# i4Ds/whisper-finetune

Hardware: AMD Instinct MI355X
Metric: audio-seconds/sec training throughput, whisper-large-v3 bf16 (higher is better)
Workload: dtype bf16; 1 GPU; whisper-large-v3 full fine-tune, AdamW, bf16 MFMA / fp32 master weights, 96 synthetic 30 s clips per GPU per step, decoder S=128, log-mel + SpecAugment on GPU, label smoothing 0.1, clip 1.0, local accumulation 1 (global window = 1); timed loop = model_utils.train_step; global_batch=96, seq_len=128, parallelism=dp1

## Files before the change

### include/wft.h

```cpp
#ifndef WFT_H
#define WFT_H

#include <stdint.h>

#ifdef __cplusplus
extern "C" {
#endif

typedef enum {
  WFT_OK = 0,
  WFT_ERR_ARG = -1,
  WFT_ERR_LAUNCH = -2,
  WFT_ERR_UNSUPPORTED = -3
} wft_status;

typedef uint16_t wft_bf16;

const char* wft_last_error(void);
const char* wft_version(void);

int wft_cast_f32_bf16(const float* src, wft_bf16* dst, int64_t n, void* stream);
int wft_cast_bf16_f32(const wft_bf16* src, float* dst, int64_t n, void* stream);
int wft_cast_pad_transpose_f32_bf16(const float* src, int64_t rows, int64_t cols,
                                    wft_bf16* dst, wft_bf16* dst_t,
// ... 90 lines not shown
int wft_gemm_nt_rank_pair_bf16(const wft_gemm_args* args0, const wft_gemm_args* args1, void* stream);
int wft_gemm_tn_rank_pair_bf16(const wft_gemm_args* args0, const wft_gemm_args* args1, void* stream);
int64_t wft_gemm_tn_workspace_bytes(const wft_gemm_args* args);

typedef struct {
  const wft_bf16* q; int64_t ldq; int64_t q_bs;
  const wft_bf16* k; int64_t ldk; int64_t k_bs;
  const wft_bf16* v; int64_t ldv; int64_t v_bs;
  wft_bf16* o; int64_t ldo; int64_t o_bs;
  float* lse;
  int B; int H; int Tq; int Tk; int causal; float scale;
  const wft_bf16* d_o; int64_t lddo; int64_t do_bs;
  float* delta;
  wft_bf16* dq; int64_t lddq; int64_t dq_bs;
  wft_bf16* dk; int64_t lddk; int64_t dk_bs;
  wft_bf16* dv; int64_t lddv; int64_t dv_bs;
  float* dq_colsum; float* dv_colsum; float* colsum_ws;
  int launch_mode; int variant; int q_prescaled;
} wft_attn_args;
int wft_attn_fwd_bf16(const wft_attn_args* args, void* stream);
int wft_attn_bwd_bf16(const wft_attn_args* args, void* stream);
int64_t wft_attn_bwd_colsum_workspace_bytes(const wft_attn_args* args);
int wft_attn_variant(const wft_attn_args* args, int which);

int wft_embed_fwd(const int64_t* tokens, const float* emb, const float* pos,
                  wft_bf16* out, int64_t B, int64_t S, int d, int64_t V, void* stream);
int wft_embed_bwd(const int64_t* tokens, const wft_bf16* dout, float* demb, float* dpos,
                  int64_t B, int64_t S, int d, int64_t V, void* stream);

int wft_ce_fwd(const wft_bf16* logits, int64_t ld, const int64_t* targets,
               int64_t rows, int64_t V, float label_smoothing,
               float* row_loss, float* row_lse, float* stats, int64_t* argmax,
               void* stream);
int wft_ce_bwd(const wft_bf16* logits, int64_t ld, const int64_t* targets,
               int64_t rows, int64_t V, float label_smoothing,
               const float* row_lse, const float* stats, const float* gscale,
               wft_bf16* dlogits, void* stream);

int wft_token_stats(const wft_bf16* logits, int64_t ld, const int64_t* targets,
                    int64_t rows, int64_t V, float* out4, int64_t* argmax, void* stream);

typedef struct {
  const wft_bf16* q; int64_t ldq;
  const wft_bf16* k_new; const wft_bf16* v_new; int64_t ld_new;
  wft_bf16* k_cache; wft_bf16* v_cache; int64_t ld_cache; int64_t cache_bs;
  wft_bf16* o; int64_t ldo;
// ... 146 lines not shown
```

### whisper-finetune_amd/csrc/attn.hip

```cpp
#include "attn_common.h"

static void attn_fill(const wft_attn_args* a, AttnP& p) {
  p.q = a->q; p.ldq = a->ldq; p.q_bs = a->q_bs;
  p.k = a->k; p.ldk = a->ldk; p.k_bs = a->k_bs;
  p.v = a->v; p.ldv = a->ldv; p.v_bs = a->v_bs;
  p.o = a->o; p.ldo = a->ldo; p.o_bs = a->o_bs;
  p.lse = a->lse;
  p.B = a->B; p.H = a->H; p.Tq = a->Tq; p.Tk = a->Tk; p.causal = a->causal;
  p.scale = a->scale;
  p.qpre = a->q_prescaled ? 1 : 0;
  p.c = p.qpre ? 1.0f : a->scale * LOG2E;
  p.ls = p.qpre ? LN2 : a->scale;
  p.d_o = a->d_o; p.lddo = a->lddo; p.do_bs = a->do_bs;
  p.delta = a->delta;
  p.dq = a->dq; p.lddq = a->lddq; p.dq_bs = a->dq_bs;
  p.dk = a->dk; p.lddk = a->lddk; p.dk_bs = a->dk_bs;
  p.dv = a->dv; p.lddv = a->lddv; p.dv_bs = a->dv_bs;
  p.cs_q = nullptr; p.cs_v = nullptr;
  static const int xcd_on = [] { const char* e = wft_dev_getenv("WFT_ATTN_XCD"); return e ? atoi(e) : 1; }();
  p.xcd = xcd_on;
}

#define ATT_CS_CHUNKS 32
__global__ __launch_bounds__(256) void attn_colsum_reduce_kernel(const float* partial0, long nrows0, float* out0,
// ... 17 lines not shown

#define ATT_ALIGNED(ptr, ld, bs) ((((uintptr_t)(ptr)) & 15) == 0 && ((ld) % 8) == 0 && ((bs) % 8) == 0)
static int attn_check(const wft_attn_args* a, bool bwd, const char* who, const char* align_msg) {
  WFT_CHECK_ARG_AS(who, a && a->q && a->k && a->v && a->o && a->lse &&
                            (!bwd || (a->d_o && a->delta && a->dq && a->dk && a->dv)),
                   "null pointer");
  WFT_CHECK_ARG_AS(who, a->B >= 1 && a->H >= 1 && a->Tq >= 1 && a->Tk >= 1, "bad shape");
  WFT_CHECK_ARG_AS(who, ATT_ALIGNED(a->q, a->ldq, a->q_bs) && ATT_ALIGNED(a->k, a->ldk, a->k_bs) &&
                            ATT_ALIGNED(a->v, a->ldv, a->v_bs) && ATT_ALIGNED(a->o, a->ldo, a->o_bs) &&
                            (!bwd || (ATT_ALIGNED(a->d_o, a->lddo, a->do_bs) && ATT_ALIGNED(a->dq, a->lddq, a->dq_bs) &&
                                      ATT_ALIGNED(a->dk, a->lddk, a->dk_bs) && ATT_ALIGNED(a->dv, a->lddv, a->dv_bs))),
                   align_msg);
  WFT_CHECK_ARG_AS(who, !a->causal || a->Tq == a->Tk, "causal attention needs Tq == Tk");
  if (!bwd) return WFT_OK;
  WFT_CHECK_ARG_AS(who, a->scale > 0.f, "scale must be positive (the row constants are -lse / scale)");
  WFT_CHECK_ARG_AS(who, (!a->dq_colsum && !a->dv_colsum && !a->colsum_ws) || (a->dq_colsum && a->dv_colsum && a->colsum_ws),
                   "dq_colsum, dv_colsum and colsum_ws go together");
  return WFT_OK;
}

static int g_attn_persistent = [] { const char* e = getenv("WFT_ATTN_PERSISTENT"); return (e && e[0] == '0') ? 0 : 1; }();
struct AttnPlan {
  bool fwd_pipe = false;
  bool dq4w = false, dkdv4w = false;
  unsigned fwd_grid = 0, dq_grid = 0, dkdv_grid = 0;
  long rows_q = 0, rows_v = 0, cs_q = 0, cs_v = 0, mid_q = 0, mid_v = 0;
  int64_t colsum_bytes = 0;
};
static unsigned attn_persistent_grid(const wft_attn_args* a, int rows, int wgs_env) {
  const bool persistent = g_attn_persistent != 0 && a->launch_mode != 1;
  const long items = (long)((rows + 255) / 256) * a->H * a->B;
  long wgs = wgs_env > 0 ? wgs_env : (persistent ? wft_num_cus() : items);
  if (wgs > items) wgs = items;
  if (((long)a->H * a->B) % 8 == 0 && wgs >= 8) wgs -= wgs % 8;
  return (unsigned)wgs;
}
static AttnPlan attn_plan(const wft_attn_args* a) {
  AttnPlan pl;
  if (!a) return pl;
  static const int dkdv_wgs_env = [] { const char* e = wft_dev_getenv("WFT_DKDV_WGS"); return e ? atoi(e) : 0; }();
  pl.fwd_pipe = wft_fwd_pipe_eligible(a);
  pl.dq4w = wft_dq4w_eligible(a);
  pl.dkdv4w = wft_dkdv4w_eligible(a);
  const unsigned grid_q = (unsigned)(((a->Tq + 127) / 128) * a->H * a->B), grid_k = (unsigned)(((a->Tk + 127) / 128) * a->H * a->B);
  pl.fwd_grid = grid_q;
  pl.dq_grid = pl.dq4w ? attn_persistent_grid(a, a->Tq, 0) : grid_q;
  pl.dkdv_grid = pl.dkdv4w ? attn_persistent_grid(a, a->Tk, dkdv_wgs_env) : grid_k;
  const long n = (long)a->H * 64;
  pl.rows_q = (long)a->B * ((a->Tq + 31) / 32);
  pl.rows_v = (long)a->B * ((a->Tk + 31) / 32);
  pl.cs_v = pl.rows_q * n;
  pl.mid_q = pl.cs_v + pl.rows_v * n;
  pl.mid_v = pl.mid_q + (long)ATT_CS_CHUNKS * n;
  pl.colsum_bytes = (pl.mid_v + (int64_t)ATT_CS_CHUNKS * n) * (int64_t)sizeof(float);
  return pl;
}

extern "C" int64_t wft_attn_bwd_colsum_workspace_bytes(const wft_attn_args* a) { return attn_plan(a).colsum_bytes; }

extern "C" int wft_attn_variant(const wft_attn_args* a, int which) {
  if (!a) return WFT_ERR_ARG;
  const AttnPlan pl = attn_plan(a);
  if (which == 0) return pl.fwd_pipe ? 2 : 1;
  if (which == 1) return pl.dq4w ? 4 : 8;
  if (which == 2) return pl.dkdv4w ? 4 : 8;
  return WFT_ERR_ARG;
}

extern "C" int wft_attn_fwd_bf16(const wft_attn_args* a, void* stream) {
  if (const int rc = attn_check(a, false, __func__, "q/k/v/o need 16-byte aligned bases and strides that are multiples of 8")) return rc;
  AttnP p;
  attn_fill(a, p);
  const AttnPlan pl = attn_plan(a);
  wft_attn_fwd_launch(p, pl.fwd_pipe, dim3(pl.fwd_grid), (hipStream_t)stream);
  WFT_CHECK_LAUNCH();
  return WFT_OK;
}

extern "C" int wft_attn_bwd_bf16(const wft_attn_args* a, void* stream) {
  if (const int rc = attn_check(a, true, __func__, "tensors need 16-byte aligned bases and strides that are multiples of 8")) return rc;
  AttnP p;
  attn_fill(a, p);
  const AttnPlan pl = attn_plan(a);
  if (a->colsum_ws) {
    p.cs_q = a->colsum_ws + pl.cs_q;
    p.cs_v = a->colsum_ws + pl.cs_v;
  }
  hipStream_t s = (hipStream_t)stream;
  int rc = WFT_OK;
  if (pl.dq4w) rc = wft_dq4w_launch(p, dim3(pl.dq_grid), s);
  else wft_attn_dq8w_launch(p, dim3(pl.dq_grid), s);
  if (rc != WFT_OK) return rc;
  rc = pl.dkdv4w ? wft_dkdv4w_launch(p, dim3(pl.dkdv_grid), s) : wft_attn_dkdv8w_launch(p, dim3(pl.dkdv_grid), s);
  if (rc != WFT_OK) return rc;
  if (p.cs_q) {
    const int n = a->H * 64;
    float* mid_q = a->colsum_ws + pl.mid_q;
// ... 10 lines not shown
```

### whisper-finetune_amd/csrc/attn_common.h

```cpp
#pragma once
#include "common.h"
#include "gemm_common.h"
#include <stdlib.h>
#include <string.h>
#define ATT_NEG (-1.0e30f)
#define ATT_TAU 8.0f
#define LOG2E 1.4426950408889634f
#define LN2 0.6931471805599453f

struct AttnP {
  const unsigned short* q; long ldq, q_bs;
  const unsigned short* k; long ldk, k_bs;
  const unsigned short* v; long ldv, v_bs;
  unsigned short* o; long ldo, o_bs;
  float* lse;
  int B, H, Tq, Tk, causal;
  float scale;
  const unsigned short* d_o; long lddo, do_bs;
  float* delta;
  unsigned short* dq; long lddq, dq_bs;
  unsigned short* dk; long lddk, dk_bs;
  unsigned short* dv; long lddv, dv_bs;
  float* cs_q;
  float* cs_v;
// ... 205 lines not shown
template <int N>
__device__ __forceinline__ float w4_acc() {
  float x;
  asm volatile("v_accvgpr_read_b32 %0, a[%1]" : "=v"(x) : "i"(N));
  return x;
}
template <int BASE>
__device__ __forceinline__ f32x16 w4_get16() {
  f32x16 v;
  v[0] = w4_acc<BASE>(); v[1] = w4_acc<BASE + 1>(); v[2] = w4_acc<BASE + 2>(); v[3] = w4_acc<BASE + 3>();
  v[4] = w4_acc<BASE + 4>(); v[5] = w4_acc<BASE + 5>(); v[6] = w4_acc<BASE + 6>(); v[7] = w4_acc<BASE + 7>();
  v[8] = w4_acc<BASE + 8>(); v[9] = w4_acc<BASE + 9>(); v[10] = w4_acc<BASE + 10>(); v[11] = w4_acc<BASE + 11>();
  v[12] = w4_acc<BASE + 12>(); v[13] = w4_acc<BASE + 13>(); v[14] = w4_acc<BASE + 14>(); v[15] = w4_acc<BASE + 15>();
  return v;
}

static inline bool attn_offsets_fit32(const wft_attn_args* a) {
  const long lim = 0x7fffffffL;
  return (long)(a->Tq + 256) * a->ldq * 2 < lim && (long)(a->Tq + 256) * a->lddo * 2 < lim && (long)(a->Tk + 256) * a->ldk * 2 < lim &&
         (long)(a->Tk + 256) * a->ldv * 2 < lim;
}
bool wft_fwd_pipe_eligible(const wft_attn_args* a);
void wft_attn_fwd_launch(const AttnP& p, bool pipe, dim3 grid, hipStream_t s);
void wft_attn_dq8w_launch(const AttnP& p, dim3 grid, hipStream_t s);
int wft_attn_dkdv8w_launch(const AttnP& p, dim3 grid, hipStream_t s);
bool wft_dq4w_eligible(const wft_attn_args* a);
int wft_dq4w_launch(const AttnP& p, dim3 grid, hipStream_t s);
bool wft_dkdv4w_eligible(const wft_attn_args* a);
int wft_dkdv4w_launch(const AttnP& p, dim3 grid, hipStream_t s);
```

### whisper-finetune_amd/whisper_finetune/engine/kernels.py

```python
from __future__ import annotations

import ctypes as C
import math
from typing import Optional

import torch

from . import lib as L

BF16 = torch.bfloat16
F32 = torch.float32

PROFILE_NT = None


def _p(t: Optional[torch.Tensor]):
    return C.c_void_p(0 if t is None else t.data_ptr())


def _chk(t: torch.Tensor, dtype, name: str):
    if t.dtype != dtype:
        raise TypeError(f"{name}: expected {dtype}, got {t.dtype}")
    if not t.is_cuda:
        raise L.WftError(f"{name}: libwft kernels need CUDA/HIP tensors (got {t.device}); there is no CPU path")
# ... 191 lines not shown
    need_ws = want_params or want_colsum
    ws = torch.empty(lib.wft_layernorm_bwd_workspace(rows, cols), dtype=torch.uint8, device=x.device) if need_ws else None
    dx = torch.empty_like(x)
    dgamma = torch.empty(cols, dtype=F32, device=x.device) if want_params else None
    dbeta = torch.empty(cols, dtype=F32, device=x.device) if want_params else None
    dxs = torch.empty(cols, dtype=F32, device=x.device) if want_colsum else None
    if mask is not None and len(mask) == 2:
        rpb, span = mask
        _chk_flag(span, 4, "span")
        L.check(lib.wft_layernorm_bwd_dspan(_p(dy), _p(x), _p(gamma), _p(mean), _p(rstd), _p(dres), _p(dx), _p(dgamma), _p(dbeta),
                                            _p(dxs), _p(ws), rows, cols, int(rpb), _p(span), L.stream_ptr()), "wft_layernorm_bwd_dspan")
    else:
        rpb, t0, t1, c0, c1 = mask if mask is not None else (0, 0, 0, 0, 0)
        L.check(
                lib.wft_layernorm_bwd(_p(dy), _p(x), _p(gamma), _p(mean), _p(rstd), _p(dres), _p(dx), _p(dgamma), _p(dbeta),
                                      _p(dxs), _p(ws), rows, cols, rpb, t0, t1, c0, c1, L.stream_ptr()),
            "wft_layernorm_bwd",
        )
    if want_colsum:
        return dx, dgamma, dbeta, dxs
    return dx, dgamma, dbeta


VARIANT = {"nt": 0, "tn": 0, "fwd": 0, "dq": 0, "dkdv": 0}
LAUNCH_OVERRIDE = [None]
LAUNCH_PERSISTENT, LAUNCH_PER_TILE = 0, 1


def set_variant(which: str, v: int) -> int:
    old = VARIANT[which]
    if v >= 0:
        VARIANT[which] = 1 if v else 0
    return old


def _launch(launch: int) -> int:
    o = LAUNCH_OVERRIDE[0]
    return int(launch) if o is None else int(o)


def _attn_variant_bits() -> int:
    return VARIANT["fwd"] | (VARIANT["dq"] << 1) | (VARIANT["dkdv"] << 2)


def gemm_nt(a, b, *, M=None, N=None, K=None, lda=None, ldb=None, out=None, out_f32=False, accumulate=False,
            bias=None, residual=None, aux=None, epilogue=L.EPI_NONE, alpha=1.0, batch=1,
            strideA=0, strideB=0, strideC=0, strideR=0, strideAux=0, ldc=None,
            valid_rows_period=0, valid_rows=0, residual_first=False, ldaux=None, ldr=None, beta=1.0, colsum=None, p_valid=0,
            launch=0, _args_only=False):
    _chk(a, BF16, "A"); _chk(b, BF16, "B")
    if M is None:
        M = a.shape[0]
    if K is None:
        K = a.shape[-1]
    if N is None:
        N = b.shape[0]
    if lda is None:
        lda = a.stride(-2) if a.dim() >= 2 else K
    if ldb is None:
        ldb = b.stride(-2)
    if out is None:
        out = torch.empty((batch * M, N) if batch > 1 else (M, N), dtype=F32 if out_f32 else BF16, device=a.device)
        if batch > 1 and strideC == 0:
            strideC = M * N
    if ldc is None:
# ... 212 lines not shown

def _tn_workspace(device, nbytes: int, slot: str = "tn") -> torch.Tensor:
    key = (device.type, device.index, slot)
    ws = _TN_WS.get(key)
    if ws is None or ws.numel() < nbytes:
        ws = torch.empty(max(nbytes, 64 << 20), dtype=torch.uint8, device=device)
        _TN_WS[key] = ws
    return ws


def _grant_workspace(args, query: str, device, slot: str) -> int:
    need = getattr(L.load(), query)(C.byref(args))
    if need > 0:
        ws = _tn_workspace(device, need, slot=slot)
        args.workspace, args.workspace_bytes = ws.data_ptr(), ws.numel()
    return need


def _attn_view(t: torch.Tensor):
    assert t.dim() == 3 and t.stride(2) == 1
    return t.data_ptr(), t.stride(1), t.stride(0)


def attn_fwd(q, k, v, n_head: int, causal: bool, scale: float, q_prescaled: bool = False, o=None, lse=None):
    for n, t in (("q", q), ("k", k), ("v", v)):
        _chk(t, BF16, n)
    B, Tq, D = q.shape
    Tk = k.shape[1]
    assert D == n_head * 64, "head_dim must be 64"
    if o is None:
        o = torch.empty((B, Tq, D), dtype=BF16, device=q.device)
    else:
        _chk(o, BF16, "o")
        assert o.shape == (B, Tq, D)
    if lse is None:
        lse = torch.empty((B, n_head, Tq), dtype=F32, device=q.device)
    else:
        _chk(lse, F32, "lse")
        assert lse.shape == (B, n_head, Tq) and lse.is_contiguous()
    a = L.AttnArgs()
    a.q, a.ldq, a.q_bs = _attn_view(q)
    a.k, a.ldk, a.k_bs = _attn_view(k)
    a.v, a.ldv, a.v_bs = _attn_view(v)
    a.o, a.ldo, a.o_bs = _attn_view(o)
    a.lse = lse.data_ptr()
    a.B, a.H, a.Tq, a.Tk, a.causal, a.scale = B, n_head, Tq, Tk, int(causal), scale
    a.variant, a.q_prescaled = _attn_variant_bits(), int(bool(q_prescaled))
    L.check(L.load().wft_attn_fwd_bf16(C.byref(a), L.stream_ptr()), "wft_attn_fwd_bf16")
    return o, lse


def attn_bwd(q, k, v, o, lse, do, n_head: int, causal: bool, scale: float, dq=None, dk=None, dv=None, colsums=None,
             q_prescaled: bool = False, launch: int = 0):
    B, Tq, D = q.shape
    Tk = k.shape[1]
    _chk(do, BF16, "do")
    if do.stride(2) != 1:
        do = do.contiguous()
    dq = torch.empty((B, Tq, D), dtype=BF16, device=q.device) if dq is None else dq
    dk = torch.empty((B, Tk, D), dtype=BF16, device=q.device) if dk is None else dk
    dv = torch.empty((B, Tk, D), dtype=BF16, device=q.device) if dv is None else dv
    delta = torch.empty((2, B, n_head, Tq), dtype=F32, device=q.device)
    a = L.AttnArgs()
    a.q, a.ldq, a.q_bs = _attn_view(q)
    a.k, a.ldk, a.k_bs = _attn_view(k)
    a.v, a.ldv, a.v_bs = _attn_view(v)
    a.o, a.ldo, a.o_bs = _attn_view(o)
    a.lse = lse.data_ptr()
    a.B, a.H, a.Tq, a.Tk, a.causal, a.scale = B, n_head, Tq, Tk, int(causal), scale
    a.d_o, a.lddo, a.do_bs = _attn_view(do)
# ... 693 lines not shown
```

### whisper-finetune_amd/whisper_finetune/engine/lib.py

```python
from __future__ import annotations

import ctypes as C
import os
from pathlib import Path

_PKG_ROOT = Path(__file__).resolve().parents[2]
LIB_PATH = Path(os.environ.get("WFT_LIB", _PKG_ROOT / "libwft.so"))

c_i64 = C.c_int64
c_vp = C.c_void_p


class GemmArgs(C.Structure):

    _fields_ = [
        ("A", c_vp), ("lda", c_i64), ("strideA", c_i64),
        ("B", c_vp), ("ldb", c_i64), ("strideB", c_i64),
        ("C", c_vp), ("ldc", c_i64), ("strideC", c_i64), ("c_is_f32", C.c_int), ("accumulate", C.c_int),
        ("bias", c_vp),
        ("residual", c_vp), ("ldr", c_i64), ("strideR", c_i64),
        ("aux", c_vp), ("ldaux", c_i64), ("strideAux", c_i64),
        ("epilogue", C.c_int), ("alpha", C.c_float),
        ("M", c_i64), ("N", c_i64), ("K", c_i64), ("batch", C.c_int),
        ("valid_rows_period", C.c_int), ("valid_rows", C.c_int),
# ... 139 lines not shown
    "wft_layernorm_bwd_dspan": [c_vp, c_vp, c_vp, c_vp, c_vp, c_vp, c_vp, c_vp, c_vp, c_vp, c_vp, c_i64, C.c_int,
                                C.c_int, c_vp, c_vp],
    "wft_gemm_nt_bf16": [C.POINTER(GemmArgs), c_vp],
    "wft_gemm_nt_variant": [C.POINTER(GemmArgs)],
    "wft_gemm_tn_segments_ok": [C.POINTER(GemmArgs)],
    "wft_gemm_nt_colsum_workspace_bytes": [C.POINTER(GemmArgs)],
    "wft_gemm_nt_splitk_workspace_bytes": [C.POINTER(GemmArgs)],
    "wft_gemm_nt_aux8_bytes": [C.POINTER(GemmArgs)],
    "wft_gemm_nt_stream_bf16": [C.POINTER(GemmArgs), c_vp],
    "wft_gemm_nt_stream_ok": [C.POINTER(GemmArgs)],
    "wft_gemm_nt_stream_workspace_bytes": [C.POINTER(GemmArgs)],
    "wft_gemm_nt_stream_q8": [C.POINTER(GemmArgs), c_vp, c_vp],
    "wft_gemm_nt_stream_q8_ok": [C.POINTER(GemmArgs)],
    "wft_gemm_nt_stream_q8_workspace_bytes": [C.POINTER(GemmArgs)],
    "wft_gemm_tn_bf16": [C.POINTER(GemmArgs), c_vp],
    "wft_gemm_tn_variant": [C.POINTER(GemmArgs)],
    "wft_gemm_nt_rank_pair_bf16": [C.POINTER(GemmArgs), C.POINTER(GemmArgs), c_vp],
    "wft_gemm_tn_rank_pair_bf16": [C.POINTER(GemmArgs), C.POINTER(GemmArgs), c_vp],
    "wft_gemm_tn_workspace_bytes": [C.POINTER(GemmArgs)],
    "wft_attn_fwd_bf16": [C.POINTER(AttnArgs), c_vp],
    "wft_attn_bwd_bf16": [C.POINTER(AttnArgs), c_vp],
    "wft_attn_bwd_colsum_workspace_bytes": [C.POINTER(AttnArgs)],
    "wft_attn_variant": [C.POINTER(AttnArgs), C.c_int],
    "wft_attn_decode_bf16": [C.POINTER(AttnDecodeArgs), c_vp],
    "wft_attn_decode_workspace_bytes": [C.POINTER(AttnDecodeArgs)],
    "wft_decode_embed": [c_vp, c_i64, c_vp, c_vp, c_vp, c_vp, C.c_int, C.c_int, C.c_int, c_i64, c_vp],
    "wft_decode_pick": [C.POINTER(DecodePickArgs), c_vp],
    "wft_attn_decode_beam_bf16": [C.POINTER(AttnDecodeBeamArgs), c_vp],
    "wft_attn_decode_beam_workspace_bytes": [C.POINTER(AttnDecodeBeamArgs)],
    "wft_decode_topk": [C.POINTER(DecodeTopkArgs), c_vp],
    "wft_decode_pick_ts": [C.POINTER(DecodePickArgs), C.POINTER(TsRules), c_vp],
    "wft_decode_topk_ts": [C.POINTER(DecodeTopkArgs), C.POINTER(TsRules), c_vp, c_i64, C.c_int, c_vp],
    "wft_beam_update": [C.POINTER(BeamUpdateArgs), c_vp],
    "wft_decode_sample": [C.POINTER(DecodePickArgs), C.POINTER(SampleRules), c_vp],
    "wft_decode_sample_ts": [C.POINTER(DecodePickArgs), C.POINTER(SampleRules), C.POINTER(TsRules), c_vp],
    "wft_attn_probs_bf16": [C.POINTER(AttnArgs), c_vp, C.c_int, c_vp, c_vp, c_vp, c_i64, c_i64, c_i64, c_vp],
    "wft_align_matrix": [c_vp, c_i64, c_i64, c_i64, c_vp, c_vp, c_vp, c_i64, c_i64, C.c_int, C.c_int, C.c_int, C.c_int, C.c_int, c_vp],
    "wft_dtw_workspace_bytes": [C.c_int, C.c_int, C.c_int],
    "wft_dtw_f32": [c_vp, c_i64, c_i64, C.c_int, C.c_int, c_vp, c_vp, C.c_int, C.c_int, C.c_int, C.c_int, c_vp, c_vp, c_i64, c_vp, c_vp,
                    c_i64, c_vp],
    "wft_word_spans": [c_vp, c_vp, c_i64, c_vp, c_vp, c_i64, c_vp, c_vp, c_i64, c_vp, c_vp, c_vp, c_vp, c_i64, C.c_int, C.c_int, c_vp],
    "wft_lang_probs": [c_vp, c_i64, c_i64, c_vp, C.c_int, c_vp, c_i64, c_vp, C.c_int, c_vp],
    "wft_mel_windows": [c_vp, c_vp, c_vp, c_vp, c_vp, c_vp, c_vp, C.c_int, C.c_int, C.c_int, C.c_int, c_vp],
    "wft_embed_fwd": [c_vp, c_vp, c_vp, c_vp, c_i64, c_i64, C.c_int, c_i64, c_vp],
    "wft_embed_bwd": [c_vp, c_vp, c_vp, c_vp, c_i64, c_i64, C.c_int, c_i64, c_vp],
    "wft_ce_fwd": [c_vp, c_i64, c_vp, c_i64, c_i64, C.c_float, c_vp, c_vp, c_vp, c_vp, c_vp],
# ... 90 lines not shown
```

Baseline: 3644 audio-s/s.

## Add persistent 4-wave hand-scheduled assembly attention forward kernel

Adds a new persistent attention forward kernel written in inline assembly. Each workgroup of four waves loops over (batch, head, query-block) items, keeping a four-slot LDS ring of K/V tiles filled by LDS-direct buffer loads. The softmax exponentials, max reductions and P·V MFMAs are interleaved, with a lazy rescale slow path taken only when the running max grows past a threshold. The next item's Q and first tiles are prefetched behind the current item's output store. It applies by default when Tq≥256 and Tk≥192, which covers the 1500-frame encoder self-attention. The cost is a large, hard-to-maintain assembly path with more risk of correctness bugs.

```diff
diff --git a/include/wft.h b/include/wft.h
--- a/include/wft.h
+++ b/include/wft.h
@@ -136,6 +136,7 @@
 int wft_attn_bwd_bf16(const wft_attn_args* args, void* stream);
 int64_t wft_attn_bwd_colsum_workspace_bytes(const wft_attn_args* args);
 int wft_attn_variant(const wft_attn_args* args, int which);
+int wft_attn_fwd_variant(const wft_attn_args* args);
 
 int wft_embed_fwd(const int64_t* tokens, const float* emb, const float* pos,
                   wft_bf16* out, int64_t B, int64_t S, int d, int64_t V, void* stream);
diff --git a/whisper-finetune_amd/csrc/attn.hip b/whisper-finetune_amd/csrc/attn.hip
--- a/whisper-finetune_amd/csrc/attn.hip
+++ b/whisper-finetune_amd/csrc/attn.hip
@@ -63,6 +63,7 @@
 static int g_attn_persistent = [] { const char* e = getenv("WFT_ATTN_PERSISTENT"); return (e && e[0] == '0') ? 0 : 1; }();
 struct AttnPlan {
   bool fwd_pipe = false;
+  bool fwd4w = false;
   bool dq4w = false, dkdv4w = false;
   unsigned fwd_grid = 0, dq_grid = 0, dkdv_grid = 0;
   long rows_q = 0, rows_v = 0, cs_q = 0, cs_v = 0, mid_q = 0, mid_v = 0;
@@ -81,10 +82,11 @@
   if (!a) return pl;
   static const int dkdv_wgs_env = [] { const char* e = wft_dev_getenv("WFT_DKDV_WGS"); return e ? atoi(e) : 0; }();
   pl.fwd_pipe = wft_fwd_pipe_eligible(a);
+  pl.fwd4w = wft_fwd4w_eligible(a);
   pl.dq4w = wft_dq4w_eligible(a);
   pl.dkdv4w = wft_dkdv4w_eligible(a);
   const unsigned grid_q = (unsigned)(((a->Tq + 127) / 128) * a->H * a->B), grid_k = (unsigned)(((a->Tk + 127) / 128) * a->H * a->B);
-  pl.fwd_grid = grid_q;
+  pl.fwd_grid = pl.fwd4w ? attn_persistent_grid(a, a->Tq, 0) : grid_q;
   pl.dq_grid = pl.dq4w ? attn_persistent_grid(a, a->Tq, 0) : grid_q;
   pl.dkdv_grid = pl.dkdv4w ? attn_persistent_grid(a, a->Tk, dkdv_wgs_env) : grid_k;
   const long n = (long)a->H * 64;
@@ -108,12 +110,22 @@
   return WFT_ERR_ARG;
 }
 
+extern "C" int wft_attn_fwd_variant(const wft_attn_args* a) {
+  if (!a) return WFT_ERR_ARG;
+  const AttnPlan pl = attn_plan(a);
+  return pl.fwd4w ? 4 : pl.fwd_pipe ? 2 : 1;
+}
+
 extern "C" int wft_attn_fwd_bf16(const wft_attn_args* a, void* stream) {
   if (const int rc = attn_check(a, false, __func__, "q/k/v/o need 16-byte aligned bases and strides that are multiples of 8")) return rc;
   AttnP p;
   attn_fill(a, p);
   const AttnPlan pl = attn_plan(a);
-  wft_attn_fwd_launch(p, pl.fwd_pipe, dim3(pl.fwd_grid), (hipStream_t)stream);
+  if (pl.fwd4w) {
+    if (const int rc = wft_fwd4w_launch(p, dim3(pl.fwd_grid), (hipStream_t)stream)) return rc;
+  } else {
+    wft_attn_fwd_launch(p, pl.fwd_pipe, dim3(pl.fwd_grid), (hipStream_t)stream);
+  }
   WFT_CHECK_LAUNCH();
   return WFT_OK;
 }
diff --git a/whisper-finetune_amd/csrc/attn_common.h b/whisper-finetune_amd/csrc/attn_common.h
--- a/whisper-finetune_amd/csrc/attn_common.h
+++ b/whisper-finetune_amd/csrc/attn_common.h
@@ -251,6 +251,8 @@
 }
 bool wft_fwd_pipe_eligible(const wft_attn_args* a);
 void wft_attn_fwd_launch(const AttnP& p, bool pipe, dim3 grid, hipStream_t s);
+bool wft_fwd4w_eligible(const wft_attn_args* a);
+int wft_fwd4w_launch(const AttnP& p, dim3 grid, hipStream_t s);
 void wft_attn_dq8w_launch(const AttnP& p, dim3 grid, hipStream_t s);
 int wft_attn_dkdv8w_launch(const AttnP& p, dim3 grid, hipStream_t s);
 bool wft_dq4w_eligible(const wft_attn_args* a);
diff --git a/whisper-finetune_amd/csrc/attn_fwd4w.hip b/whisper-finetune_amd/csrc/attn_fwd4w.hip
--- /dev/null
+++ b/whisper-finetune_amd/csrc/attn_fwd4w.hip
@@ -0,0 +1,627 @@
+#include "attn_common.h"
+#define F4_BUF 20480
+#define F4_QT 10240
+#define F4_LDS (4 * F4_BUF + 4 * F4_QT)
+#define F4_ASM_MACROS R"ASM(
+; registers: S(g,qb,kb) v[g+32qb+16kb..+15], g = 128 / 192; P(qb,ks) v[32+16qb+4ks..+3]; -m(qb) x 16: v[64+16qb..+15];
+; m(qb) v[96+qb], l(qb) v[98+qb], row-sum partials v[100+2qb], v[101+2qb]; v104-v107 maximum partials, v108-v110 half exchange / tmax,
+; v111 d, v112 alpha, v113-v115, v120-v126 scratch, v116 K row read base (tile j+1), v117 V transposed read base (tile j), v118 mask
+; limit, v119 -1e30;  O^T(qb,db) a[32qb+16db..+15], Q rows QF(qb,s) a[64+16qb+4s..+3], K rows KF(kb,s) a[96+16kb+4s..+3],
+; V^T(ks,db) a[128+8ks+4db..+3]
+.macro F4_PV n, qb
+  v_mfma_f32_32x32x16_bf16 a[32*\qb+16*((\n)%%2):32*\qb+16*((\n)%%2)+15], a[128+8*((\n)/2)+4*((\n)%%2):128+8*((\n)/2)+4*((\n)%%2)+3], v[32+16*\qb+4*((\n)/2):32+16*\qb+4*((\n)/2)+3], a[32*\qb+16*((\n)%%2):32*\qb+16*((\n)%%2)+15]
+.endm
+.macro F4_S n, qb, g
+  .if ((\n) %% 4) == 0
+    v_mfma_f32_32x32x16_bf16 v[\g+32*\qb+16*((\n)/4):\g+32*\qb+16*((\n)/4)+15], a[96+4*(\n):96+4*(\n)+3], a[64+16*\qb+4*((\n)%%4):64+16*\qb+4*((\n)%%4)+3], v[64+16*\qb:64+16*\qb+15]
+  .else
+    v_mfma_f32_32x32x16_bf16 v[\g+32*\qb+16*((\n)/4):\g+32*\qb+16*((\n)/4)+15], a[96+4*(\n):96+4*(\n)+3], a[64+16*\qb+4*((\n)%%4):64+16*\qb+4*((\n)%%4)+3], v[\g+32*\qb+16*((\n)/4):\g+32*\qb+16*((\n)/4)+15]
+  .endif
+.endm
+; K row read i (0..7): key block i/4, k-step i%%4
+.macro F4_RDK i, rb
+  ds_read_b128 a[96+4*(\i):96+4*(\i)+3], \rb offset:512*((\i)/4)+32*((\i)%%4)
+.endm
+; transposed V read m (0..15) in the order the P.V MFMAs consume them: fragment m/2 = (ks, db) = (m/4, (m/2)%%2), half t = m%%2
+.macro F4_RDV m, tb
+  ds_read_b64_tr_b16 a[128+8*((\m)/4)+4*(((\m)/2)%%2)+2*((\m)%%2):128+8*((\m)/4)+4*(((\m)/2)%%2)+2*((\m)%%2)+1], \tb offset:10240+5152*((\m)%%2)+256*((\m)/4)+64*(((\m)/2)%%2)
+.endm
+.macro F4_ADVANCE
+  s_add_u32 s40, s40, s56
+  s_addc_u32 s41, s41, 0
+  s_sub_u32 s42, s42, s56
+  s_cselect_b32 s42, 0, s42
+  s_add_u32 s44, s44, s57
+  s_addc_u32 s45, s45, 0
+  s_sub_u32 s46, s46, s57
+  s_cselect_b32 s46, 0, s46
+.endm
+; step i (0..3) of this wave's share of one tile -> the ring slot at LDS offset \boff: pieces 2 wave, 2 wave + 1 of K (0, 1) and V (2, 3)
+.macro F4_DMA i, boff
+  .if (\i) == 0
+    s_add_u32 m0, s58, \boff
+    s_nop 0
+    buffer_load_dwordx4 %[voK0], s[40:43], 0 offen lds
+  .elseif (\i) == 1
+    s_add_u32 m0, s59, \boff
+    s_nop 0
+    buffer_load_dwordx4 %[voK1], s[40:43], 0 offen lds
+  .elseif (\i) == 2
+    s_add_u32 m0, s58, \boff
+    s_add_u32 m0, m0, 10240
+    s_nop 0
+    buffer_load_dwordx4 %[voV0], s[44:47], 0 offen lds
+  .else
+    s_add_u32 m0, s59, \boff
+    s_add_u32 m0, m0, 10240
+    s_nop 0
+    buffer_load_dwordx4 %[voV1], s[44:47], 0 offen lds
+  .endif
+.endm
+; exponential step e (0..16) of the unit whose 32 scores are v[U..U+31] (key order): exponentials of elements 2e, 2e+1; the row-sum
+; adds and the pack of step e-1 one step behind (a v_exp result is not read by the next instruction).  0 + p is exact, so the first
+; add of each partial takes two exponentials
+.macro F4_STEP e, U, pf, ls
+  .if (\e) < 16
+    .if att_pre == 0
+      v_mul_f32 v[\U+2*(\e)], %[c], v[\U+2*(\e)]
+      v_mul_f32 v[\U+2*(\e)+1], %[c], v[\U+2*(\e)+1]
+    .endif
+    v_exp_f32 v[\U+2*(\e)], v[\U+2*(\e)]
+    v_exp_f32 v[\U+2*(\e)+1], v[\U+2*(\e)+1]
+  .endif
+  .if (\e) == 2
+    v_add_f32 v[\ls], v[\U], v[\U+2]
+    v_add_f32 v[\ls+1], v[\U+1], v[\U+3]
+  .elseif (\e) > 2
+    v_add_f32 v[\ls], v[\ls], v[\U+2*(\e)-2]
+    v_add_f32 v[\ls+1], v[\ls+1], v[\U+2*(\e)-1]
+  .endif
+  .if (\e) >= 1
+    v_cvt_pk_bf16_f32 v[\pf+(\e)-1], v[\U+2*(\e)-2], v[\U+2*(\e)-1]
+  .endif
+.endm
+; l += xhalf_sum(ls0 + ls1)
+.macro F4_LFLUSH ls, l
+  v_add_f32 v122, v[\ls], v[\ls+1]
+  v_mov_b32 v120, v122
+  v_mov_b32 v121, v122
+  s_nop 1
+  v_permlane32_swap_b32 v120, v121
+  s_nop 1
+  v_add_f32 v122, v120, v121
+  v_add_f32 v[\l], v[\l], v122
+.endm
+; operation k (0..15) of the in-lane maximum over v[U..U+31] (the tree of att_max32) -> v104
+.macro F4_MAX k, U
+  .if (\k) < 4
+    v_max3_f32 v[104+(\k)], v[\U+16*((\k)/2)+3*((\k)%%2)], v[\U+16*((\k)/2)+3*((\k)%%2)+1], v[\U+16*((\k)/2)+3*((\k)%%2)+2]
+  .elseif (\k) < 12
+    v_max3_f32 v[104+(\k)%%4], v[104+(\k)%%4], v[\U+16*(((\k)%%4)/2)+6+2*((\k)%%2)+4*((\k)/4-1)], v[\U+16*(((\k)%%4)/2)+7+2*((\k)%%2)+4*((\k)/4-1)]
+  .elseif (\k) == 12
+    v_max3_f32 v104, v104, v[\U+14], v[\U+15]
+  .elseif (\k) == 13
+    v_max3_f32 v106, v106, v[\U+30], v[\U+31]
+  .elseif (\k) == 14
+    v_max_f32 v104, v104, v105
+  .else
+    v_max3_f32 v104, v104, v106, v107
+  .endif
+.endm
+; the last tile: keys at or past Tk -> -1e30 (v118 = Tk - first key of the tile - 4 h; element i of a unit is key 32 (i/16) + 8 ((i%%16)/4) + i%%4 + 4 h)
+.macro F4_MASK U
+  s_cmp_eq_u32 s77, 0
+  s_cbranch_scc1 8f
+  .set f4_i, 0
+  .rept 32
+    v_cmp_gt_i32 vcc, v118, 32*(f4_i/16)+8*((f4_i%%16)/4)+(f4_i%%4)
+    v_cndmask_b32 v[\U+f4_i], v119, v[\U+f4_i], vcc
+    .set f4_i, f4_i+1
+  .endr
+8:
+.endm
+; half iteration (j, qb).  gV: generation of tile j, gM: of tiles j-1 / j+1; first: tile 0 (nothing to finish, no P.V, the rescale is
+; unconditional); last: tile n-1 (mask; no S, no K reads, no LDS-DMA); sl / bl: labels of the slow path and of its return point
+.macro F4_HALF gV, gM, qb, first, last, sl, bl
+  .if \last
+    F4_MASK \gV+32*\qb
+  .endif
+  .set f4_s, 0
+  .rept 16
+    ; counted LDS waits at even slots, for the fragments of this slot and the next: V^T fragment f is followed by the 2 (7 - f) later
+    ; transposed reads and the K row reads of slots 0 .. f-1; K row read i (slot i) is used in slot 8 + i
+    .if \qb == 0 && f4_s < 8 && \first == 0 && (f4_s %% 2) == 0
+      .if \last
+        s_waitcnt lgkmcnt(12-2*f4_s)
+      .else
+        s_waitcnt lgkmcnt(12-f4_s)
+      .endif
+    .endif
+    .if \qb == 0 && f4_s >= 8 && \last == 0 && (f4_s %% 2) == 0
+      s_waitcnt lgkmcnt(14-f4_s)
+    .endif
+    .if f4_s < 8
+      .if \first == 0
+        F4_PV f4_s, \qb
+      .endif
+    .else
+      .if \last == 0
+        F4_S f4_s-8, \qb, \gM
+      .endif
+    .endif
+    .if f4_s < 8
+      .if \qb == 0 && \first == 0
+        F4_STEP 8+f4_s, \gM+32, 48, 102
+      .elseif \qb == 1
+        F4_STEP 8+f4_s, \gV, 32, 100
+      .endif
+      .if f4_s < 5
+        F4_MAX 3*f4_s, \gV+32*\qb
+        F4_MAX 3*f4_s+1, \gV+32*\qb
+        F4_MAX 3*f4_s+2, \gV+32*\qb
+      .elseif f4_s == 5
+        F4_MAX 15, \gV+32*\qb
+        v_mov_b32 v109, v104
+      .elseif f4_s == 6
+        ; (half exchange: v104 <- the lower half's value, v109 <- the upper half's, in every lane; the copy, the swap and the maximum
+        ; are a slot apart, so the permlane hazards of att_xhalf are covered by the instructions between them; tile 0's first half has none)
+        .if \first && \qb == 0
+          s_nop 1
+        .endif
+        v_permlane32_swap_b32 v104, v109
+      .else
+        .if \first && \qb == 0
+          s_nop 1
+        .endif
+        v_max_f32 v110, v104, v109
+        .if \first
+          s_branch \sl\()f
+        .else
+          .if att_pre == 0
+            v_mul_f32 v113, %[c], v110
+            v_cmp_lt_f32 vcc, 0x41000000, v113
+          .else
+            v_cmp_lt_f32 vcc, 0x41000000, v110
+          .endif
+          s_cbranch_vccnz \sl\()f
+        .endif
+\bl:
+      .endif
+    .else
+      .if \qb == 1 || \first == 0
+        ; the other block's unit ends: its last adds and pack, then l += xhalf_sum(ls0 + ls1) with the copy, the swap and the adds a
+        ; slot apart (partials v[100+2(1-qb)], +1; l = v[98+(1-qb)])
+        .if f4_s == 8
+          .if \qb == 0
+            F4_STEP 16, \gM+32, 48, 102
+          .else
+            F4_STEP 16, \gV, 32, 100
+          .endif
+          v_add_f32 v122, v[100+2*(1-\qb)], v[101+2*(1-\qb)]
+          v_mov_b32 v121, v122
+        .elseif f4_s == 9
+          v_permlane32_swap_b32 v122, v121
+        .elseif f4_s == 10
+          v_add_f32 v122, v122, v121
+          v_add_f32 v[98+(1-\qb)], v[98+(1-\qb)], v122
+        .endif
+      .endif
+      F4_STEP f4_s-8, \gV+32*\qb, 32+16*\qb, 100+2*\qb
+    .endif
+    .if \qb == 0 && f4_s < 8 && \last == 0
+      F4_RDK f4_s, v116
+    .endif
+    .if \qb == 1 && f4_s >= 8
+      F4_RDV 2*(f4_s-8), v117
+      F4_RDV 2*(f4_s-8)+1, v117
+    .endif
+    .if \qb == 0 && \last == 0 && f4_s >= 8 && f4_s < 12
+      F4_DMA f4_s-8, s76
+    .endif
+    .if \qb == 0 && \last == 0 && f4_s == 12
+      F4_ADVANCE
+    .endif
+    .set f4_s, f4_s+1
+  .endr
+.endm
+; the rescale of block qb in front of tile j's exponentials (unit v[U..U+31]): d = first ? tmax : max(tmax, 0), alpha = exp2(-d c),
+; m += d, l *= alpha, s -= d, O *= alpha, C operand = -m.  The P.V MFMAs of tile j-1 were issued in full: drain them first
+.macro F4_SLOW U, qb, first, sl, bl
+\sl:
+  s_nop 15
+  s_nop 15
+  .if \first
+    v_mov_b32 v111, v110
+  .else
+    v_max_f32 v111, 0, v110
+  .endif
+  .if att_pre == 0
+    v_mul_f32_e64 v113, -v111, %[c]
+    v_exp_f32 v112, v113
+  .else
+    v_exp_f32_e64 v112, -v111
+  .endif
+  v_add_f32 v[96+\qb], v[96+\qb], v111
+  v_xor_b32 v113, 0x80000000, v[96+\qb]
+  .set f4_i, 0
+  .rept 16
+    v_mov_b32 v[64+16*\qb+f4_i], v113
+    .set f4_i, f4_i+1
+  .endr
+  .set f4_i, 0
+  .rept 32
+    v_sub_f32 v[\U+f4_i], v[\U+f4_i], v111
+    .set f4_i, f4_i+1
+  .endr
+  v_mul_f32 v[98+\qb], v[98+\qb], v112
+  .set f4_i, 0
+  .rept 8
+    v_accvgpr_read_b32 v123, a[32*\qb+4*f4_i]
+    v_accvgpr_read_b32 v124, a[32*\qb+4*f4_i+1]
+    v_accvgpr_read_b32 v125, a[32*\qb+4*f4_i+2]
+    v_accvgpr_read_b32 v126, a[32*\qb+4*f4_i+3]
+    v_mul_f32 v123, v123, v112
+    v_mul_f32 v124, v124, v112
+    v_mul_f32 v125, v125, v112
+    v_mul_f32 v126, v126, v112
+    v_accvgpr_write_b32 a[32*\qb+4*f4_i], v123
+    v_accvgpr_write_b32 a[32*\qb+4*f4_i+1], v124
+    v_accvgpr_write_b32 a[32*\qb+4*f4_i+2], v125
+    v_accvgpr_write_b32 a[32*\qb+4*f4_i+3], v126
+    .set f4_i, f4_i+1
+  .endr
+  s_nop 4
+  s_branch \bl\()b
+.endm
+; one tile: tile j+1 has landed for every wave (this wave's four pieces of tile j+2 may still fly), tile j-1's slot is free -> tile
+; j+3 goes into it; the two halves; the ring moves on.  k0..k3: the halves' label pairs
+.macro F4_ITER gV, gM, first, last, k0, k1, k2, k3
+  s_waitcnt vmcnt(4)
+  s_barrier
+  F4_HALF \gV, \gM, 0, \first, \last, \k0, \k1
+  F4_HALF \gV, \gM, 1, \first, \last, \k2, \k3
+  s_mov_b32 s67, s63
+  s_mov_b32 s63, s64
+  s_mov_b32 s64, s65
+  s_mov_b32 s65, s76
+  s_mov_b32 s76, s67
+  v_add_u32 v116, s64, %[rb]
+  v_add_u32 v117, s63, %[tb]
+.endm
+; behind the last tile: the rest of block 1's exponentials under P.V(n-1) of block 0, then P.V(n-1) of block 1
+.macro F4_TAIL gV
+  .set f4_s, 0
+  .rept 8
+    .if (f4_s %% 2) == 0
+      s_waitcnt lgkmcnt(12-2*f4_s)
+    .endif
+    F4_PV f4_s, 0
+    F4_STEP 8+f4_s, \gV+32, 48, 102
+    .set f4_s, f4_s+1
+  .endr
+  F4_STEP 16, \gV+32, 48, 102
+  F4_LFLUSH 102, 99
+  s_nop 1
+  .set f4_s, 0
+  .rept 8
+    F4_PV f4_s, 1
+    .set f4_s, f4_s+1
+  .endr
+.endm
+; descriptors: K s[40:43], V s[44:47] (tile strides s56, s57), Q s[68:71]; this wave's Q transit area s53; LDS-DMA destinations inside a
+; ring slot: piece 2 wave (s58), 2 wave + 1 (s59); ring slot offsets: tile j s63, j+1 s64, j+2 s65, j+3 s76
+.macro F4_SRD_INIT
+  s_mov_b64 s[40:41], %[bK]
+  s_lshr_b32 s61, %[stK], 6
+  s_sub_u32 s62, %[tk], 1
+  s_mul_i32 s42, s62, s61
+  s_add_u32 s42, s42, 128
+  s_mov_b32 s43, 0x20000
+  s_mov_b64 s[44:45], %[bV]
+  s_lshr_b32 s61, %[stV], 6
+  s_mul_i32 s46, s62, s61
+  s_add_u32 s46, s46, 128
+  s_mov_b32 s47, 0x20000
+  s_mov_b32 s56, %[stK]
+  s_mov_b32 s57, %[stV]
+  s_mov_b64 s[68:69], %[bQ]
+  s_sub_u32 s62, %[tq], 1
+  s_mul_i32 s70, s62, %[ldq2]
+  s_add_u32 s70, s70, 128
+  s_mov_b32 s71, 0x20000
+  s_mul_i32 s53, %[wave], )ASM" W4_STR(F4_QT) R"ASM(
+  s_add_u32 s53, s53, 4*)ASM" W4_STR(F4_BUF) R"ASM(
+  s_add_u32 s53, s53, %[lds0]
+  s_lshl_b32 s61, %[wave], 1
+  s_mul_i32 s58, s61, 1280
+  s_lshr_b32 s62, s61, 1
+  s_lshl_b32 s62, s62, 4
+  s_add_u32 s58, s58, s62
+  s_add_u32 s58, s58, %[lds0]
+  s_add_u32 s59, s58, 1344
+  s_mov_b32 s63, 0
+  s_mov_b32 s64, )ASM" W4_STR(F4_BUF) R"ASM(
+  s_mov_b32 s65, 2*)ASM" W4_STR(F4_BUF) R"ASM(
+  s_mov_b32 s76, 3*)ASM" W4_STR(F4_BUF) R"ASM(
+.endm
+; Q rows of this wave's 64 queries -> its transit area in the piece layout (rows past Tq arrive as zeros)
+.macro F4_TRANSIT
+  .set f4_i, 0
+  .rept 8
+    s_mul_i32 s61, %[ldq2], (f4_i%%2)+4*(f4_i/2)
+    s_add_u32 m0, s53, f4_i*1280+64*(f4_i%%2)+16*(f4_i/2)
+    v_add_u32 v[114+(f4_i%%2)], s61, %[voQ]
+    s_nop 0
+    buffer_load_dwordx4 v[114+(f4_i%%2)], s[68:71], 0 offen lds
+    .set f4_i, f4_i+1
+  .endr
+.endm
+; key tiles 0, 1, 2 -> ring slots 0, 1, 2 (sources end up three tiles on)
+.macro F4_STAGE3
+  s_nop 4
+  F4_DMA 0, s63
+  F4_DMA 1, s63
+  F4_DMA 2, s63
+  F4_DMA 3, s63
+  F4_ADVANCE
+  s_nop 4
+  F4_DMA 0, s64
+  F4_DMA 1, s64
+  F4_DMA 2, s64
+  F4_DMA 3, s64
+  F4_ADVANCE
+  s_nop 4
+  F4_DMA 0, s65
+  F4_DMA 1, s65
+  F4_DMA 2, s65
+  F4_DMA 3, s65
+  F4_ADVANCE
+.endm
+)ASM"
+#define F4_ASM_PURGE R"ASM(
+.purgem F4_PV
+.purgem F4_S
+.purgem F4_RDK
+.purgem F4_RDV
+.purgem F4_ADVANCE
+.purgem F4_DMA
+.purgem F4_STEP
+.purgem F4_LFLUSH
+.purgem F4_MAX
+.purgem F4_MASK
+.purgem F4_HALF
+.purgem F4_SLOW
+.purgem F4_ITER
+.purgem F4_TAIL
+.purgem F4_SRD_INIT
+.purgem F4_TRANSIT
+.purgem F4_STAGE3
+)ASM"
+#define F4_CLOBBER_A "a0", "a1", "a2", "a3", "a4", "a5", "a6", "a7", "a8", "a9", W4_A8(1), W4_A8(2), W4_A8(3), W4_A8(4), W4_A8(5), W4_A8(6), W4_A8(7), W4_A8(8), W4_A8(9), W4_A8(10), W4_A8(11), W4_A8(12), W4_A8(13), W4_A8(14), W4_A8(15)
+
+template <bool PRE>
+__global__ __launch_bounds__(256) void attn_fwd4w_kernel(AttnP p) {
+  extern __shared__ __attribute__((aligned(16))) char smem[];
+  const int tid = threadIdx.x, lane = tid & 63;
+  const int wave = __builtin_amdgcn_readfirstlane(tid >> 6);
+  const int r = lane & 31, h = lane >> 5;
+  const int nqb = (p.Tq + 255) >> 8;
+  const int ngrp = p.H * p.B;
+  const bool xcd_mode = ((ngrp & 7) == 0) && p.xcd && ((gridDim.x & 7) == 0);
+  const int xcd = xcd_mode ? (int)(blockIdx.x & 7) : 0;
+  const int w0 = xcd_mode ? (int)(blockIdx.x >> 3) : (int)blockIdx.x;
+  const int wstep = xcd_mode ? (int)(gridDim.x >> 3) : (int)gridDim.x;
+  const int nitems = (xcd_mode ? ngrp >> 3 : ngrp) * nqb;
+  if (w0 >= nitems) return;
+  const unsigned lds0 = __builtin_amdgcn_readfirstlane(lds_addr_of(smem));
+  const int c = r & 15, pidr = (c & 1) | ((c >> 2) << 1);
+  const unsigned rb = lds0 + pidr * W4_PIECE + 64 * (pidr & 1) + 16 * (pidr >> 1) + (2 * (r >> 4) + ((c >> 1) & 1)) * 128 + h * 16;
+  const int g4 = lane >> 4, i16 = lane & 15, pidt = ((i16 >> 2) & 1) | ((g4 >> 1) << 1);
+  const unsigned tb = lds0 + pidt * W4_PIECE + 64 * (pidt & 1) + 16 * (pidt >> 1) + ((i16 >> 3) & 1) * 128 + 32 * (g4 & 1) + 8 * (i16 & 3);
+  const int slot = lane >> 3, ch = lane & 7;
+  auto krow = [&](int pid) { return (pid & 1) + 4 * (pid >> 1) + 2 * (slot & 1) + 16 * (slot >> 1); };
+  const unsigned voK0 = (unsigned)(krow(2 * wave) * (int)p.ldk + ch * 8) * 2u, voK1 = (unsigned)(krow(2 * wave + 1) * (int)p.ldk + ch * 8) * 2u;
+  const unsigned voV0 = (unsigned)(krow(2 * wave) * (int)p.ldv + ch * 8) * 2u, voV1 = (unsigned)(krow(2 * wave + 1) * (int)p.ldv + ch * 8) * 2u;
+  auto sg64 = [](unsigned long long x) {
+    const unsigned lo = __builtin_amdgcn_readfirstlane((unsigned)x), hi = __builtin_amdgcn_readfirstlane((unsigned)(x >> 32));
+    return ((unsigned long long)hi << 32) | lo;
+  };
+  const unsigned tq = __builtin_amdgcn_readfirstlane((unsigned)p.Tq), tk = __builtin_amdgcn_readfirstlane((unsigned)p.Tk);
+  const unsigned ldq2 = __builtin_amdgcn_readfirstlane((unsigned)p.ldq * 2u);
+  const unsigned stK = __builtin_amdgcn_readfirstlane((unsigned)p.ldk * 128u), stV = __builtin_amdgcn_readfirstlane((unsigned)p.ldv * 128u);
+  const unsigned ntile = __builtin_amdgcn_readfirstlane((unsigned)((p.Tk + 63) >> 6));
+  const int lim0 = p.Tk - 64 * ((p.Tk + 63) / 64 - 1) - 4 * h;
+  const unsigned cbits = __builtin_amdgcn_readfirstlane(__builtin_bit_cast(unsigned, p.c));
+  const unsigned wv = (unsigned)wave;
+
+  struct Item {
+    int b, hd, qw0;
+    unsigned long long bQ, bK, bV;
+    unsigned voQ;
+  };
+  auto coords = [&](int t, Item& x) {
+    const int g = xcd_mode ? (t / nqb) * 8 + xcd : t / nqb;
+    x.hd = g % p.H;
+    x.b = g / p.H;
+    x.qw0 = (t % nqb) * 256 + wave * 64;
+    x.bQ = sg64((unsigned long long)(p.q + (long)x.b * p.q_bs + x.hd * 64));
+    x.bK = sg64((unsigned long long)(p.k + (long)x.b * p.k_bs + x.hd * 64));
+    x.bV = sg64((unsigned long long)(p.v + (long)x.b * p.v_bs + x.hd * 64));
+    x.voQ = (unsigned)((x.qw0 + 2 * (slot & 1) + 16 * (slot >> 1)) * (int)p.ldq + ch * 8) * 2u;
+  };
+  Item cur;
+  coords(w0, cur);
+
+  for (int t = w0; t < nitems; t += wstep) {
+  const int b = cur.b, hd = cur.hd, qw0 = cur.qw0;
+  const unsigned first = __builtin_amdgcn_readfirstlane((unsigned)(t == w0));
+  float mo0, mo1, lo0, lo1;
+  asm volatile(".set att_pre, %c[pre]\n" F4_ASM_MACROS R"ASM(
+    F4_SRD_INIT
+    s_sub_u32 s66, %[ntile], 2      ; loop counter: tiles 1 .. n-2
+    s_and_b32 s77, %[tk], 63        ; != 0: the last tile is ragged
+    s_cmp_eq_u32 %[first], 0
+    s_cbranch_scc1 2f
+    ; ---- first item of this workgroup: its Q rows and key tiles 0, 1, 2 are requested here ...
+    F4_TRANSIT
+    F4_STAGE3
+    s_branch 3f
+2:
+    ; ---- ... later ones found them requested by the prefetch block behind the previous item (below): only the descriptors move on
+    F4_ADVANCE
+    F4_ADVANCE
+    F4_ADVANCE
+3:
+    ; ---- (under the loads) O^T, m, l and the C operands start from zero
+    .set f4_i, 0
+    .rept 64
+      v_accvgpr_write_b32 a[f4_i], 0
+      .set f4_i, f4_i+1
+    .endr
+    .set f4_i, 64
+    .rept 36
+      v_mov_b32 v[f4_i], 0
+      .set f4_i, f4_i+1
+    .endr
+    v_mov_b32 v119, 0xf149f2ca      ; -1e30
+    v_mov_b32 v118, %[lim0]
+    v_mov_b32 v116, %[rb]
+    s_sub_u32 s61, s53, %[lds0]
+    v_add_u32 v114, s61, %[rb]
+    s_cmp_eq_u32 %[first], 0
+    s_cbranch_scc0 7f
+    s_waitcnt vmcnt(0)             ; later items: the previous item's O stores were issued behind the prefetch, so everything drains
+7:
+    s_waitcnt vmcnt(8)             ; Q rows and tile 0 (tiles 1, 2: eight pieces may still be in flight)
+    s_barrier
+    ; Q row fragments (lane (r, h): query 32 qb + r, columns 16 s + 8 h .. + 8) from the transit area -> a[64:95]
+    .set f4_i, 0
+    .rept 8
+      ds_read_b128 a[64+4*f4_i:64+4*f4_i+3], v114 offset:512*(f4_i/4)+32*(f4_i%%4)
+      .set f4_i, f4_i+1
+    .endr
+    ; ---- tile 0: K row fragments, S^T -> generation 128
+    .set f4_i, 0
+    .rept 8
+      F4_RDK f4_i, v116
+      .set f4_i, f4_i+1
+    .endr
+    s_waitcnt lgkmcnt(0)
+    .set f4_i, 0
+    .rept 8
+      F4_S f4_i, 0, 128
+      .set f4_i, f4_i+1
+    .endr
+    .set f4_i, 0
+    .rept 8
+      F4_S f4_i, 1, 128
+      .set f4_i, f4_i+1
+    .endr
+    v_add_u32 v116, s64, %[rb]
+    v_add_u32 v117, s63, %[tb]
+    s_nop 15
+    s_nop 15
+    F4_ITER 128, 192, 1, 0, 30, 31, 32, 33
+4:
+    F4_ITER 192, 128, 0, 0, 34, 35, 36, 37
+    s_sub_u32 s66, s66, 1
+    s_cmp_eq_u32 s66, 0
+    s_cbranch_scc1 5f
+    F4_ITER 128, 192, 0, 0, 38, 39, 40, 41
+    s_sub_u32 s66, s66, 1
+    s_cmp_eq_u32 s66, 0
+    s_cbranch_scc1 6f
+    s_branch 4b
+5:
+    ; ---- the last tile (keys past Tk are switched off element by element), generation 128
+    F4_ITER 128, 192, 0, 1, 42, 43, 44, 45
+    F4_TAIL 128
+    s_branch 9f
+6:
+    ; ---- the same, generation 192
+    F4_ITER 192, 128, 0, 1, 46, 47, 48, 49
+    F4_TAIL 192
+    s_branch 9f
+    ; ---- the rescale slow paths, one per decision point
+    F4_SLOW 128, 0, 1, 30, 31
+    F4_SLOW 160, 1, 1, 32, 33
+    F4_SLOW 192, 0, 0, 34, 35
+    F4_SLOW 224, 1, 0, 36, 37
+    F4_SLOW 128, 0, 0, 38, 39
+    F4_SLOW 160, 1, 0, 40, 41
+    F4_SLOW 128, 0, 0, 42, 43
+    F4_SLOW 160, 1, 0, 44, 45
+    F4_SLOW 192, 0, 0, 46, 47
+    F4_SLOW 224, 1, 0, 48, 49
+9:
+    s_waitcnt vmcnt(0)
+    s_nop 15
+    s_nop 15
+    v_mov_b32 %[mo0], v96
+    v_mov_b32 %[mo1], v97
+    v_mov_b32 %[lo0], v98
+    v_mov_b32 %[lo1], v99
+  )ASM" F4_ASM_PURGE
+               : [mo0] "=&v"(mo0), [mo1] "=&v"(mo1), [lo0] "=&v"(lo0), [lo1] "=&v"(lo1)
+               : [rb] "v"(rb), [tb] "v"(tb), [voK0] "v"(voK0), [voK1] "v"(voK1), [voV0] "v"(voV0), [voV1] "v"(voV1), [voQ] "v"(cur.voQ),
+                 [lim0] "v"(lim0), [bK] "s"(sg64(cur.bK)), [bV] "s"(sg64(cur.bV)), [bQ] "s"(sg64(cur.bQ)), [tq] "s"(tq), [tk] "s"(tk),
+                 [ldq2] "s"(ldq2), [stK] "s"(stK), [stV] "s"(stV), [ntile] "s"(ntile), [c] "s"(cbits), [lds0] "s"(lds0), [wave] "s"(wv),
+                 [first] "s"(first), [pre] "n"(PRE ? 1 : 0)
+               : "memory", "vcc", "scc", F4_CLOBBER_A, W4_CLOBBER_V, W4_CLOBBER_S);
+
+  Item nx;
+  const bool more = t + wstep < nitems;
+  if (more) {
+    coords(t + wstep, nx);
+    asm volatile(".set att_pre, 0\n" F4_ASM_MACROS R"ASM(
+      s_barrier
+      F4_SRD_INIT
+      F4_TRANSIT
+      F4_STAGE3
+    )ASM" F4_ASM_PURGE
+                 :
+                 : [rb] "v"(rb), [tb] "v"(tb), [c] "s"(cbits), [voK0] "v"(voK0), [voK1] "v"(voK1), [voV0] "v"(voV0), [voV1] "v"(voV1),
+                   [voQ] "v"(nx.voQ), [bK] "s"(sg64(nx.bK)), [bV] "s"(sg64(nx.bV)), [bQ] "s"(sg64(nx.bQ)), [tq] "s"(tq), [tk] "s"(tk),
+                   [ldq2] "s"(ldq2), [stK] "s"(stK), [stV] "s"(stV), [lds0] "s"(lds0), [wave] "s"(wv)
+                 : "memory", "scc", "v114", "v115", W4_CLOBBER_S);
+  }
+
+  auto row16 = [&](const f32x16& acc, int m2, float mul) {
+    const unsigned x0 = pack2bf(acc[8 * m2] * mul, acc[8 * m2 + 1] * mul), x1 = pack2bf(acc[8 * m2 + 2] * mul, acc[8 * m2 + 3] * mul);
+    const unsigned y0 = pack2bf(acc[8 * m2 + 4] * mul, acc[8 * m2 + 5] * mul), y1 = pack2bf(acc[8 * m2 + 6] * mul, acc[8 * m2 + 7] * mul);
+    const auto s0 = __builtin_amdgcn_permlane32_swap(x0, y0, false, false), s1 = __builtin_amdgcn_permlane32_swap(x1, y1, false, false);
+    u32x4 o = {s0[0], s1[0], s0[1], s1[1]};
+    return o;
+  };
+  auto store = [&](auto qbc, float m, float l) {
+    constexpr int qb = decltype(qbc)::value;
+    const int qi = qw0 + 32 * qb + r;
+    f32x16 oacc[2];
+    oacc[0] = w4_get16<32 * qb>(); oacc[1] = w4_get16<32 * qb + 16>();
+    const float inv = 1.0f / l;
+    unsigned short* orow = p.o + (long)b * p.o_bs + (long)qi * p.ldo + hd * 64;
+#pragma unroll
+    for (int db = 0; db < 2; ++db)
+#pragma unroll
+      for (int m2 = 0; m2 < 2; ++m2) {
+        const u32x4 pk = row16(oacc[db], m2, inv);
+        if (qi < p.Tq) *(u32x4*)(orow + 32 * db + 8 * (2 * m2 + h)) = pk;
+      }
+    if (qi < p.Tq && h == 0 && p.lse) p.lse[((long)b * p.H + hd) * p.Tq + qi] = m * p.ls + __logf(l);
+  };
+  store(IntC<0>{}, mo0, lo0);
+  store(IntC<1>{}, mo1, lo1);
+  if (more) cur = nx;
+  }
+}
+
+bool wft_fwd4w_eligible(const wft_attn_args* a) {
+  static const int min_tq = [] { const char* e = wft_dev_getenv("WFT_FWD4W_MIN_TQ"); return e ? atoi(e) : 256; }();
+  const long lim = 0x7fffffffL;
+  const bool fit = (long)(a->Tq + 256) * a->ldq * 2 < lim && (long)(a->Tk + 256) * a->ldk * 2 < lim && (long)(a->Tk + 256) * a->ldv * 2 < lim;
+  return wft_fwd_pipe_eligible(a) && !(a->variant & 8) && a->Tq >= min_tq && a->Tk >= 192 && fit;
+}
+int wft_fwd4w_launch(const AttnP& p, dim3 grid, hipStream_t s) {
+  return !p.qpre ? wft_launch_lds<attn_fwd4w_kernel<false>>(grid, dim3(256), F4_LDS, s, p)
+                 : wft_launch_lds<attn_fwd4w_kernel<true>>(grid, dim3(256), F4_LDS, s, p);
+}
diff --git a/whisper-finetune_amd/whisper_finetune/engine/kernels.py b/whisper-finetune_amd/whisper_finetune/engine/kernels.py
--- a/whisper-finetune_amd/whisper_finetune/engine/kernels.py
+++ b/whisper-finetune_amd/whisper_finetune/engine/kernels.py
@@ -237,7 +237,7 @@
     return dx, dgamma, dbeta
 
 
-VARIANT = {"nt": 0, "tn": 0, "fwd": 0, "dq": 0, "dkdv": 0}
+VARIANT = {"nt": 0, "tn": 0, "fwd": 0, "dq": 0, "dkdv": 0, "fwd4w": 0}
 LAUNCH_OVERRIDE = [None]
 LAUNCH_PERSISTENT, LAUNCH_PER_TILE = 0, 1
 
@@ -255,7 +255,7 @@
 
 
 def _attn_variant_bits() -> int:
-    return VARIANT["fwd"] | (VARIANT["dq"] << 1) | (VARIANT["dkdv"] << 2)
+    return VARIANT["fwd"] | (VARIANT["dq"] << 1) | (VARIANT["dkdv"] << 2) | (VARIANT["fwd4w"] << 3)
 
 
 def gemm_nt(a, b, *, M=None, N=None, K=None, lda=None, ldb=None, out=None, out_f32=False, accumulate=False,
@@ -514,7 +514,7 @@
     return t.data_ptr(), t.stride(1), t.stride(0)
 
 
-def attn_fwd(q, k, v, n_head: int, causal: bool, scale: float, q_prescaled: bool = False, o=None, lse=None):
+def attn_fwd(q, k, v, n_head: int, causal: bool, scale: float, q_prescaled: bool = False, o=None, lse=None, launch: int = 0):
     for n, t in (("q", q), ("k", k), ("v", v)):
         _chk(t, BF16, n)
     B, Tq, D = q.shape
@@ -537,7 +537,7 @@
     a.o, a.ldo, a.o_bs = _attn_view(o)
     a.lse = lse.data_ptr()
     a.B, a.H, a.Tq, a.Tk, a.causal, a.scale = B, n_head, Tq, Tk, int(causal), scale
-    a.variant, a.q_prescaled = _attn_variant_bits(), int(bool(q_prescaled))
+    a.variant, a.q_prescaled, a.launch_mode = _attn_variant_bits(), int(bool(q_prescaled)), _launch(launch)
     L.check(L.load().wft_attn_fwd_bf16(C.byref(a), L.stream_ptr()), "wft_attn_fwd_bf16")
     return o, lse
 
diff --git a/whisper-finetune_amd/whisper_finetune/engine/lib.py b/whisper-finetune_amd/whisper_finetune/engine/lib.py
--- a/whisper-finetune_amd/whisper_finetune/engine/lib.py
+++ b/whisper-finetune_amd/whisper_finetune/engine/lib.py
@@ -185,6 +185,7 @@
     "wft_attn_bwd_bf16": [C.POINTER(AttnArgs), c_vp],
     "wft_attn_bwd_colsum_workspace_bytes": [C.POINTER(AttnArgs)],
     "wft_attn_variant": [C.POINTER(AttnArgs), C.c_int],
+    "wft_attn_fwd_variant": [C.POINTER(AttnArgs)],
     "wft_attn_decode_bf16": [C.POINTER(AttnDecodeArgs), c_vp],
     "wft_attn_decode_workspace_bytes": [C.POINTER(AttnDecodeArgs)],
     "wft_decode_embed": [c_vp, c_i64, c_vp, c_vp, c_vp, c_vp, C.c_int, C.c_int, C.c_int, c_i64, c_vp],
```

Result: no change. 3679 audio-s/s (median of 6 runs) (+1.0%).
